# oxfordcontrol/Clarabel.rs

Measured on NVIDIA H100. Metric: ipm_iterations_per_sec, higher is better.
Workload: dtype f64

## Files before the change

clarabel.rs_b200/csrc/ldl.cu:

```cuda
#include <cuda_runtime.h>
#include <dlfcn.h>

#include <cmath>
#include <cstdio>
#include <cstring>
#include <algorithm>
#include <thread>
#include <vector>

#include "../../include/clarabel_b200.h"
#include "ldl_device.h"
#include "symbolic.h"
#include "vec.cuh"

namespace cb {

std::atomic<unsigned long long> g_launches{0};

typedef struct ncclComm* cb_ncclComm_t;
typedef struct { char internal[128]; } cb_ncclUniqueId;
struct NcclApi {
  void* lib = nullptr;
  int (*GetUniqueId)(cb_ncclUniqueId*) = nullptr;
  int (*CommInitRank)(cb_ncclComm_t*, int, cb_ncclUniqueId, int) = nullptr;
// ... 10 lines not shown
  void* h = dlopen(libpath && *libpath ? libpath : "libnccl.so.2", RTLD_NOW | RTLD_GLOBAL);
  if (!h) { std::fprintf(stderr, "[clarabel_b200] dlopen(%s) failed: %s\n", libpath ? libpath : "libnccl.so.2", dlerror()); return nullptr; }
  api.GetUniqueId = (int (*)(cb_ncclUniqueId*))dlsym(h, "ncclGetUniqueId");
  api.CommInitRank = (int (*)(cb_ncclComm_t*, int, cb_ncclUniqueId, int))dlsym(h, "ncclCommInitRank");
  api.AllGather = (int (*)(const void*, void*, size_t, int, cb_ncclComm_t, cudaStream_t))dlsym(h, "ncclAllGather");
  api.CommDestroy = (int (*)(cb_ncclComm_t))dlsym(h, "ncclCommDestroy");
  api.GetErrorString = (const char* (*)(int))dlsym(h, "ncclGetErrorString");
  if (!api.GetUniqueId || !api.CommInitRank || !api.AllGather || !api.CommDestroy) return nullptr;
  api.lib = h;
  return &api;
}



template <int NT>
__global__ void __launch_bounds__(NT) k_factor_level(LDLDev d, int task_base, int smem_cap) {
  extern __shared__ double sm[];
  __shared__ double s_inv;
  __shared__ double sD[CB_MAX_PANEL];
  const int tid = threadIdx.x;
  const int lane = tid & 31, warp = tid >> 5, nwarp = NT >> 5;
  const int s = d.level_tasks[task_base + blockIdx.x];
  const int f = d.sn_first[s];
  const int ns = d.sn_first[s + 1] - f;
  const long long rp = d.sn_rowptr[s];
  const int nr = (int)(d.sn_rowptr[s + 1] - rp);
  const int ld = ns + nr;
  double* __restrict__ P = d.L + d.panel_off[s];
  double* __restrict__ U = d.U + d.upd_off[s];
  const long long psz = (long long)ld * ns;
  const bool use_sm = psz <= (long long)smem_cap;
  double* W = use_sm ? sm : P;

  for (long long i = tid; i < psz; i += NT) W[i] = 0.0;
  for (int b = warp; b < nr; b += nwarp)
    for (int a = b + lane; a < nr; a += 32) U[(long long)b * nr + a] = 0.0;
  __syncthreads();

  for (long long e = d.asm_ptr[s] + tid; e < d.asm_ptr[s + 1]; e += NT)
    W[d.asm_dst[e]] = d.vals[d.asm_src[e]];
  __syncthreads();

  for (long long ci = d.child_ptr[s]; ci < d.child_ptr[s + 1]; ci++) {
    const int c = d.child_list[ci];
    const long long crp = d.sn_rowptr[c];
    const int nrc = (int)(d.sn_rowptr[c + 1] - crp);
    const double* __restrict__ Uc = d.U + d.upd_off[c];
    const int* __restrict__ relc = d.rel + crp;
    for (int b = warp; b < nrc; b += nwarp) {
      const int rb = relc[b];
      for (int a = b + lane; a < nrc; a += 32) {
        const int ra = relc[a];
        const double v = Uc[(long long)b * nrc + a];
        if (rb < ns) W[(long long)rb * ld + ra] += v;
        else U[(long long)(rb - ns) * nr + (ra - ns)] += v;
      }
    }
    __syncthreads();
  }

  for (int j = 0; j < ns; j++) {
    if (tid == 0) {
      double dj = W[(long long)j * ld + j];
      if (d.reg_enable) {
        const double sg = (double)d.dsigns[f + j];
        if (dj * sg < d.reg_eps) { dj = d.reg_delta * sg; atomicAdd(&d.status[ST_REGCOUNT], 1); }
      }
      if (dj == 0.0) atomicExch(&d.status[ST_ZEROPIV], 1);
      if (dj > 0.0) atomicAdd(&d.status[ST_POSINERTIA], 1);
      const double inv = 1.0 / dj;
      if (!isfinite(inv)) atomicExch(&d.status[ST_NONFINITE], 1);
      d.D[f + j] = dj;
      d.Dinv[f + j] = inv;
      W[(long long)j * ld + j] = dj;
      s_inv = inv;
      sD[j] = dj;
    }
    __syncthreads();
    const double inv = s_inv;
    const double* __restrict__ cj = W + (long long)j * ld;
    for (int k = j + 1 + warp; k < ns; k += nwarp) {
      const double wk = cj[k] * inv;
      double* __restrict__ ck = W + (long long)k * ld;
      for (int i = k + lane; i < ld; i += 32) ck[i] -= cj[i] * wk;
    }
    __syncthreads();
    double* cjw = W + (long long)j * ld;
    for (int i = j + 1 + tid; i < ld; i += NT) cjw[i] *= inv;
  }
  __syncthreads();

  for (int b = warp; b < nr; b += nwarp) {
    for (int a = b + lane; a < nr; a += 32) {
      double acc = 0.0;
      for (int k = 0; k < ns; k++) {
        const double* __restrict__ ck = W + (long long)k * ld + ns;
        acc += ck[a] * (ck[b] * sD[k]);
      }
      U[(long long)b * nr + a] -= acc;
    }
  }
  if (use_sm) {
    for (long long i = tid; i < psz; i += NT) P[i] = W[i];
  }
}

__global__ void __launch_bounds__(256) k_factor_leaf1(LDLDev d, int task_base, int count) {
  const int i = blockIdx.x * blockDim.x + threadIdx.x;
  const bool on = i < count;
  int pos = 0, reg = 0;
  if (on) {
    const int s = d.level_tasks[task_base + i];
    const int f = d.sn_first[s];
    const long long rp = d.sn_rowptr[s];
    const int nr = (int)(d.sn_rowptr[s + 1] - rp);
    const int ld = 1 + nr;
    double* __restrict__ P = d.L + d.panel_off[s];
    double* __restrict__ U = d.U + d.upd_off[s];
    for (int a = 0; a < ld; a++) P[a] = 0.0;
    for (long long e = d.asm_ptr[s]; e < d.asm_ptr[s + 1]; e++) P[d.asm_dst[e]] = d.vals[d.asm_src[e]];
    double dj = P[0];
    if (d.reg_enable) {
      const double sg = (double)d.dsigns[f];
      if (dj * sg < d.reg_eps) { dj = d.reg_delta * sg; reg = 1; }
    }
    if (dj == 0.0) atomicExch(&d.status[ST_ZEROPIV], 1);
    pos = dj > 0.0 ? 1 : 0;
    const double inv = 1.0 / dj;
    if (!isfinite(inv)) atomicExch(&d.status[ST_NONFINITE], 1);
    d.D[f] = dj;
    d.Dinv[f] = inv;
    P[0] = dj;
    for (int a = 1; a < ld; a++) P[a] *= inv;
    for (int b = 0; b < nr; b++) {
      const double t = P[1 + b] * dj;
      for (int a = b; a < nr; a++) {
        double acc = 0.0;
        acc += P[1 + a] * t;
        U[(long long)b * nr + a] = 0.0 - acc;
      }
    }
  }
  const unsigned mp = __ballot_sync(0xffffffffu, pos != 0), mr = __ballot_sync(0xffffffffu, reg != 0);
  if ((threadIdx.x & 31) == 0) {
    if (mp) atomicAdd(&d.status[ST_POSINERTIA], __popc(mp));
    if (mr) atomicAdd(&d.status[ST_REGCOUNT], __popc(mr));
  }
}

__global__ void k_permute_in(int n, const int* __restrict__ perm, const double* __restrict__ b,
                             double* __restrict__ xp) {
  int k = blockIdx.x * blockDim.x + threadIdx.x;
  if (k < n) xp[k] = b[perm[k]];
}

__device__ __forceinline__ unsigned long long df_gtime() {
#ifdef CB_EMU
  return 0;
#else
  unsigned long long t;
  asm volatile("mov.u64 %0, %%globaltimer;" : "=l"(t));
// ... 117 lines not shown
  if (tid == 0) {
    if (c_reg) atomicAdd(&d.status[ST_REGCOUNT], c_reg);
    if (c_pos) atomicAdd(&d.status[ST_POSINERTIA], c_pos);
    if (c_zero) atomicExch(&d.status[ST_ZEROPIV], 1);
    if (c_nonf) atomicExch(&d.status[ST_NONFINITE], 1);
  }
  for (int b = warp; b < nr; b += nwarp)
    for (int a = b + lane; a < nr; a += 32) {
      double acc = 0.0;
      for (int k = 0; k < ns; k++) {
        const double* ck = W + (long long)k * ld + ns;
        acc += ck[a] * (ck[b] * sD[k]);
      }
      U[(long long)b * nr + a] -= acc;
    }
  if (use_sm) for (long long i = tid; i < psz; i += DF_NT) P[i] = W[i];
}

#define DF_DCAP 32
#define DF_REC_INTS ((int)(sizeof(DFChildRec) / sizeof(int)))
#define DF_REC_INT(r, field) (reinterpret_cast<const int*>(r)[offsetof(DFChildRec, field) / sizeof(int)])

template <int NH>
__device__ __forceinline__ void df_add_child(const LDLDev& d, const DFChildRec& ch, double* dst, int rowoff,
                                             int rstride, int coloff, int cstride) {
  const int lane = threadIdx.x & 31, warp = threadIdx.x >> 5;
  const int* __restrict__ relc = d.rel + ch.relp;
  const double* Uc = d.U + ch.uoff;
  __syncwarp();
  if (ch.contig == 3) {
// ... 303 lines not shown
        if (jj < nj) {
          const double* lk = sA + (jb + jj) * CB_PB_LD + jb;
#pragma unroll
          for (int j2 = jj + 1; j2 < JB; j2++) t[j2] -= t[jj] * lk[j2];
        }
      }
#pragma unroll
      for (int jj = 0; jj < JB; jj++) if (jj < nj) prow[(jb + jj) * DF_RB] = t[jj] * sDinv[jb + jj];
    }
  }
  __syncthreads();
  const int nrow = r1 - r0;
  for (int idx = tid; idx < ns * DF_RB; idx += DF_NT) {
    const int j = idx / DF_RB, rr = idx - j * DF_RB;
    if (rr < nrow) P[(long long)j * ld + g0 + rr] = sR[idx];
  }
}

__device__ void dff_tile(const LDLDev& d, const DFFactor& q, const DFTask& tk, double* sm, int* s_desc, int* s_ed, double* s_ev) {
  double* sAt = sm;
  double* sBt = sm + TS * TS;
  double* sC = sm + 2 * TS * TS;
  double* sD = sC + TS * (TS + 1);
  const int tid = threadIdx.x;
  const int ti = tk.a, tj = tk.b, ns = tk.ns, nr = tk.nr, f = tk.f;
  const int ld = ns + nr;
  const double* P = d.L + tk.poff;
  double* U = d.U + tk.uoff;
  const int i0 = ti * TS, j0 = tj * TS;
  const int ni = min(TS, nr - i0), nj = min(TS, nr - j0);
// ... 134 lines not shown
#endif
      if (rr < ni && cc < nj && (i0 + rr >= j0 + cc))
        U[(long long)(j0 + cc) * nr + (i0 + rr)] = (use_sc ? creg[i][j] + sC[rr * (TS + 1) + cc] : creg[i][j]) - prod;
    }
  }
#undef OWN_R
#undef OWN_C
}

__global__ void __launch_bounds__(DF_NT, 2) k_factor_df(LDLDev d, DFFactor q) {
  extern __shared__ __align__(16) double dfsm[];
  __shared__ __align__(16) int s_desc[DF_DCAP * DF_REC_INTS];
  __shared__ __align__(16) int s_task[16];
  __shared__ int s_ed[DF_ENT_FAST];
  __shared__ double s_ev[DF_ENT_FAST];
  const int tid = threadIdx.x;
  if (tid == 0) df_cur_qi = -1;
  for (;;) {
    __syncthreads();
    if (tid == 0) {
      if (q.trace && df_cur_qi >= 0) q.trace[10 * (size_t)df_cur_qi + 2] = df_gtime();
      const int qi = atomicAdd(q.qhead, 1);
      df_cur_qi = qi < q.ntask ? qi : -1;
      if (q.trace && df_cur_qi >= 0) {
        unsigned smid = 0;
#ifndef CB_EMU
        asm volatile("mov.u32 %0, %%smid;" : "=r"(smid));
#endif
        q.trace[10 * (size_t)qi] = df_gtime();
        q.trace[10 * (size_t)qi + 3] = smid;
// ... 11 lines not shown
      __syncthreads();
      dff_small(d, s, dfsm, nullptr);
      __syncthreads();
      if (tid == 0) { __threadfence(); df_front_complete(q, s); }
    } else if (kind == 1) {
      if (tid == 0) { df_wait_zero(q.pend + s); __threadfence(); if (q.trace) q.trace[10 * (size_t)qi + 1] = df_gtime(); }
      __syncthreads();
      dff_diag(d, q, tk, dfsm, s_desc, s_ed, s_ev);
      __syncthreads();
      if (tid == 0) { __threadfence(); atomicExch(q.diag_done + s, 1); }
    } else if (kind == 2) {
      if (tid == 0) { df_wait_zero(q.pend + s); __threadfence(); if (q.trace) q.trace[10 * (size_t)qi + 1] = df_gtime(); }
      __syncthreads();
      dff_rows(d, q, tk, dfsm, s_desc, s_ed, s_ev);
      __syncthreads();
      if (tid == 0) { __threadfence(); atomicSub(q.rows_left + s, 1); }
    } else {
      if (tid == 0) { df_wait_zero(q.rows_left + s); __threadfence(); if (q.trace) q.trace[10 * (size_t)qi + 1] = df_gtime(); }
      __syncthreads();
      dff_tile(d, q, tk, dfsm, s_desc, s_ed, s_ev);
      __syncthreads();
      if (tid == 0) {
        __threadfence();
        if (atomicSub(q.tiles_left + s, 1) == 1) df_front_complete(q, s);
      }
    }
  }
}

__global__ void k_update_values(double* __restrict__ vals, const int* __restrict__ idx,
                                const double* __restrict__ v, long long len) {
// ... 159 lines not shown
  CK(upload(&dff.big_pos, fp.big_pos));
  CK(upload(&dff.tile_base, fp.tile_base));
  CK(cudaFuncSetAttribute(k_factor_df, cudaFuncAttributeMaxDynamicSharedMemorySize, DF_SMEM_DOUBLES * 8));
  int occ = 0;
  CK(cudaOccupancyMaxActiveBlocksPerMultiprocessor(&occ, k_factor_df, DF_NT, (size_t)DF_SMEM_DOUBLES * 8));
  dff_grid = nsm * std::max(1, occ);
  dff_nsup4 = 4 * (size_t)S.nsup;
  if (std::getenv("CB_DF_TRACE") && dff.ntask > 0) {
    h_dff_tasks = fp.tasks;
    CK(cudaMalloc((void**)&dff.trace, (size_t)dff.ntask * 10 * sizeof(unsigned long long)));
    CK(cudaMemset(dff.trace, 0, (size_t)dff.ntask * 10 * sizeof(unsigned long long)));
  }

  const int nt = (int)sp.tasks.size();
  sv_nwide = (int)sp.wide.size();
  sv_wide_runs = std::move(sp.wide_runs);
  sv_nleaf1 = (int)sp.leaf1.size(); sv_nleafn = (int)sp.leafn.size(); sv_nleafw = (int)sp.leafw.size();
  sv_leafw_nrmax = sp.leafw_nrmax;
  sv_leafw_grid = sv_nleafw;
  sv_ntask_owned = sp.ntask_owned;
  CK(upload(&dev.gat_ptr, sp.gat_ptr));
  CK(upload(&dev.gat_src, sp.gat_src));
  CK(upload(&d_sv_wide, sp.wide));
  CK(upload(&d_sv_leaf1, sp.leaf1));
  CK(upload(&d_sv_leafn, sp.leafn));
  CK(upload(&d_sv_leafw, sp.leafw));
  CK(upload(&sv.fronts, sp.fronts));
  CK(upload(&sv.front2task, sp.front2task));
  CK(upload(&sv.parent, S.sn_parent));
  CK(upload(&sv.tasks, sp.tasks));
  sv_ninit = sp.cnt_init.size();
  sv_nzero = (size_t)nt + 2 * (size_t)S.nsup + 2;
  CK(upload(&d_sv_init, sp.cnt_init));
  CK(cudaMalloc((void**)&d_sv_cnt, (sv_ninit + sv_nzero) * sizeof(int)));
  sv.pend = d_sv_cnt; sv.fleft = d_sv_cnt + nt; sv.bleft = sv.fleft + S.nsup;
  sv.tdone = d_sv_cnt + sv_ninit; sv.ydone = sv.tdone + nt; sv.done = sv.ydone + S.nsup; sv.qhead = sv.done + S.nsup;
  sv.bpart_stride = (long long)(sp.nslots ? sp.nslots : 1) * CB_PB_MAXNS;
  CK(cudaMalloc((void**)&sv.bpart, (size_t)2 * sv.bpart_stride * sizeof(double)));
// ... 28 lines not shown

void LDLObject::release() {
  cudaSetDevice(device);
  for (auto& w : d_shard_segs) for (auto& p : w) if (p) { cudaFree(p); p = nullptr; }
  for (int* p : d_shard_xidx) if (p) cudaFree(p);
  d_shard_xidx.clear();
  if (nccl_comm) { if (NcclApi* a = nccl_api(nullptr)) a->CommDestroy((cb_ncclComm_t)nccl_comm); nccl_comm = nullptr; }
  if (d_xsend) { cudaFree(d_xsend); d_xsend = nullptr; }
  if (d_xrecv) { cudaFree(d_xrecv); d_xrecv = nullptr; }
  xbuf_cap = 0;
  auto fr = [](const void* p) { if (p) cudaFree((void*)p); };
  fr(dev.sn_first); fr(dev.sn_rowptr); fr(dev.sn_rows); fr(dev.child_ptr); fr(dev.child_list);
  fr(dev.rel); fr(dev.panel_off); fr(dev.upd_off); fr(dev.asm_ptr); fr(dev.asm_src);
  fr(dev.asm_dst); fr(dev.level_tasks); fr(dev.perm); fr(dev.dsigns); fr(dev.vals); fr(dev.L);
  fr(dev.U); fr(dev.D); fr(dev.Dinv); fr(dev.u); fr(dev.status); fr(d_xp); fr(d_bx);
  fr(d_tmp_idx); fr(d_tmp_val); fr(d_tmp_sgn); fr(sv.tasks); fr(sv.fronts); fr(sv.front2task); fr(sv.parent); fr(sv.bpart); fr(sv.trace); fr(d_sv_cnt); fr(d_sv_init); fr(d_sv_wide); fr(d_sv_leaf1); fr(d_sv_leafn); fr(d_sv_leafw); fr(d_xp2); fr(d_u2); fr(dff.tasks); fr(dff.recs); fr(d_dff_init); fr(d_dff_cnt); fr(dff.qhead); fr(dff.parent); fr(dff.big_pos); fr(dff.tile_base); fr(dff.trace); fr(dev.gat_ptr); fr(dev.gat_src); fr(dev.sc_panel_src); fr(dev.sc_panel_dst); fr(dev.sc_tile_src); fr(dev.sc_tile_dst);
  if (h_status) cudaFreeHost(h_status);
  if (ev0) cudaEventDestroy(ev0);
  if (ev1) cudaEventDestroy(ev1);
  for (auto& e : ev_leaf) if (e) { cudaEventDestroy(e); e = nullptr; }
  if (stream_a) { cudaStreamDestroy(stream_a); stream_a = nullptr; }
  if (stream_b) { cudaStreamDestroy(stream_b); stream_b = nullptr; }
  if (stream) cudaStreamDestroy(stream);
}

int LDLObject::refactor_level0() {
  CK(cudaMemsetAsync(dev.status, 0, ST_COUNT * sizeof(int), stream));
  CK(cudaMemcpyAsync(d_dff_cnt, d_dff_init, dff_nsup4 * sizeof(int), cudaMemcpyDeviceToDevice, stream));
  CK(cudaMemsetAsync(dff.qhead, 0, sizeof(int), stream));
  g_launches += plan.size();
  for (const LaunchSeg& g : plan) {
    if (g.leaf1) k_factor_leaf1<<<(g.count + 255) / 256, 256, 0, stream>>>(dev, g.base, g.count);
    else if (g.threads == 64)
      k_factor_level<64><<<g.count, 64, (size_t)g.smem_doubles * 8, stream>>>(dev, g.base, g.smem_doubles);
    else
      k_factor_level<256><<<g.count, 256, (size_t)g.smem_doubles * 8, stream>>>(dev, g.base, g.smem_doubles);
  }
  return CLDL_OK;
}

int LDLObject::refactor_async() {
  if (sharded()) return has_transport() ? refactor_sharded() : CLDL_E_ARG;
  CK(cudaSetDevice(device));
  if (int rc = refactor_level0()) return rc;
  g_launches++;
  k_factor_df<<<dff_grid, DF_NT, (size_t)DF_SMEM_DOUBLES * 8, stream>>>(dev, dff);
  invert_pivots();
  CK(cudaGetLastError());
  CK(cudaMemcpyAsync(h_status, dev.status, ST_COUNT * sizeof(int), cudaMemcpyDeviceToHost, stream));
  factored = true;
  return CLDL_OK;
}

void LDLObject::invert_pivots() {
  if (!sv_nwide) return;
  g_launches++;
  for (size_t g = 0; g + 2 < sv_wide_runs.size(); g += 2) {
    const int first = sv_wide_runs[g], cnt = sv_wide_runs[g + 2] - first, ns = sv_wide_runs[g + 1];
    k_invert_pivots<<<cnt, 64, (size_t)ns * (ns + 1) * sizeof(double), stream>>>(dev, d_sv_wide + first, cnt);
  }
}

int LDLObject::sync_status() {
  CK(cudaSetDevice(device));
  CK(cudaStreamSynchronize(stream));
  regularize_count = (uint64_t)h_status[ST_REGCOUNT];
  positive_inertia = (uint64_t)h_status[ST_POSINERTIA];
  if (dff.trace) {
    std::vector<unsigned long long> tr((size_t)dff.ntask * 10);
    CK(cudaMemcpy(tr.data(), dff.trace, tr.size() * sizeof(unsigned long long), cudaMemcpyDeviceToHost));
    if (FILE* fp = std::fopen(std::getenv("CB_DF_TRACE"), "wb")) {
      const long long nt = dff.ntask;
      std::fwrite(&nt, sizeof(nt), 1, fp);
      std::fwrite(h_dff_tasks.data(), sizeof(DFTask), (size_t)nt, fp);
      std::fwrite(tr.data(), sizeof(unsigned long long), tr.size(), fp);
// ... 104 lines not shown
    q.ntask = dff_ntask_owned;
    g_launches++;
    k_factor_df<<<dff_grid, DF_NT, (size_t)DF_SMEM_DOUBLES * 8, stream>>>(dev, q);
    CK(cudaGetLastError());
    CK(cudaMemcpyAsync(h_status, dev.status, ST_COUNT * sizeof(int), cudaMemcpyDeviceToHost, stream));
    CK(cudaStreamSynchronize(stream));
    shard_count_owned[0] = (uint64_t)h_status[ST_REGCOUNT];
    shard_count_owned[1] = (uint64_t)h_status[ST_POSINERTIA];
    factored = false;
    return CLDL_OK;
  }
  h_phase_start[0] = dff_ntask_owned;
  CK(cudaMemcpyAsync(dff.qhead, &h_phase_start[0], sizeof(int), cudaMemcpyHostToDevice, stream));
  g_launches++;
  k_factor_df<<<dff_grid, DF_NT, (size_t)DF_SMEM_DOUBLES * 8, stream>>>(dev, dff);
  invert_pivots();
  CK(cudaGetLastError());
  CK(cudaMemcpyAsync(h_status, dev.status, ST_COUNT * sizeof(int), cudaMemcpyDeviceToHost, stream));
  factored = true;
  return CLDL_OK;
}

int LDLObject::solve_phase_async(double* d_x, const double* d_b, int phase) {
  if (!sharded()) return CLDL_E_ARG;
  if (!factored) return CLDL_E_NOT_FACTORED;
  CK(cudaSetDevice(device));
  SVPlan qv = sv;
  SVRhs r;
  r.xp[0] = r.xp[1] = d_xp; r.u[0] = r.u[1] = dev.u; r.out[0] = r.out[1] = d_x;
  if (phase == 0) {
    g_launches++;
// ... 300 lines not shown
  info->nnzL_stored = (uint64_t)o.S.nnzL_stored;
  info->regularize_count = o.regularize_count;
  info->positive_inertia = o.positive_inertia;
  info->n_supernodes = (uint64_t)o.S.nsup;
  info->n_levels = (uint64_t)o.S.nlevels;
  info->flops = o.S.flops_stored;
  info->ordering_used = o.S.ordering_used;
}

int cldl_get_perm(const cldl_t* h, uint64_t* perm_out) {
  if (!h || !perm_out) return CLDL_E_ARG;
  for (int k = 0; k < h->obj.n; k++) perm_out[k] = (uint64_t)h->obj.S.perm[k];
  return CLDL_OK;
}

int cldl_update_values_dev(cldl_t* h, const int32_t* d_index, const double* d_values, uint64_t len) {
  if (!h) return CLDL_E_ARG;
  if (len == 0) return CLDL_OK;
  LDLObject& o = h->obj;
  if (cudaSetDevice(o.device) != cudaSuccess) return CLDL_E_CUDA;
  cb::k_update_values<<<(unsigned)((len + 255) / 256), 256, 0, o.stream>>>(o.dev.vals, d_index, d_values, (long long)len);
  return CLDL_OK;
}

int cldl_set_values_dev(cldl_t* h, const double* d_nzval) {
  if (!h) return CLDL_E_ARG;
  LDLObject& o = h->obj;
  if (cudaSetDevice(o.device) != cudaSuccess) return CLDL_E_CUDA;
  return cudaMemcpyAsync(o.dev.vals, d_nzval, (size_t)o.nnzA * sizeof(double), cudaMemcpyDeviceToDevice, o.stream) == cudaSuccess
             ? CLDL_OK : CLDL_E_CUDA;
// ... 72 lines not shown
```

clarabel.rs_b200/csrc/ldl_device.h:

```cpp
#pragma once
#include <cuda_runtime.h>

#include <cstdint>
#include <cstdio>
#include <thread>
#include <vector>

#include "../../include/clarabel_b200.h"
#include "symbolic.h"
#include "ldl_plan.h"
#include "ldl_solve_plan.h"

#define CB_MAX_PANEL 128
#define CB_PB_LD 66

namespace cb {

struct ncclComm;

enum { ST_REGCOUNT = 0, ST_ZEROPIV = 1, ST_POSINERTIA = 2, ST_NONFINITE = 3, ST_COUNT = 8 };

struct LDLDev {
  const int* sn_first = nullptr;
  const long long* sn_rowptr = nullptr;
// ... 31 lines not shown
  int* pend = nullptr;
  int* diag_done = nullptr;
  int* rows_left = nullptr;
  int* tiles_left = nullptr;
  int* qhead = nullptr;
  const int* parent = nullptr;
  const int* big_pos = nullptr;
  const int* tile_base = nullptr;
  unsigned long long* trace = nullptr;
};


class LDLObject {
 public:
  SVPlan sv;
  int *d_sv_init = nullptr, *d_sv_cnt = nullptr, *d_sv_wide = nullptr, *d_sv_leaf1 = nullptr, *d_sv_leafn = nullptr, *d_sv_leafw = nullptr;
  size_t sv_ninit = 0, sv_nzero = 0, sv_smem[2] = {0, 0};
  int sv_cap = 0, sv_nwide = 0, sv_nleaf1 = 0, sv_nleafn = 0, sv_nleafw = 0, sv_leafw_nrmax = 0, sv_leafw_grid = 1, sv_ntask_owned = 0;
  std::vector<SVTask> h_sv_tasks;
  std::vector<int> sv_wide_runs;
  int sv_configure();
  int sv_occupancy();
  int sv_reset();
  void sv_sweep(bool fwd, int nrhs, const SVPlan& q, const SVRhs& r);
  void sv_leaves(bool fwd, int nrhs, const SVRhs& r);
  void invert_pivots();
  DFFactor dff;
  int *d_dff_init = nullptr, *d_dff_cnt = nullptr;
  std::vector<DFTask> h_dff_tasks;
  int dff_grid = 0;
  size_t dff_nsup4 = 0;
  int sv_grid = 0;
  bool use_dataflow = true;
  int n = 0;
  int64_t nnzA = 0;
  int device = 0;
  cldl_opts opts{};
  Symbolic S;
  LDLDev dev;
  std::vector<LaunchSeg> plan;
  std::thread big_alloc;
// ... 70 lines not shown
```

clarabel.rs_b200/csrc/ldl_plan.cpp:

```cpp
#include "ldl_plan.h"

#include <algorithm>
#include <thread>

namespace cb {

namespace {

int ns_of(const Symbolic& S, int s) { return S.sn_first[s + 1] - S.sn_first[s]; }
int nr_of(const Symbolic& S, int s) { return (int)(S.sn_rowptr[s + 1] - S.sn_rowptr[s]); }

bool is_big(const Symbolic& S, int s) { return nr_of(S, s) >= CB_BIG_NR && ns_of(S, s) <= CB_PB_MAXNS; }

std::vector<char> queued(const QueueOrder& q, int nsup) {
  std::vector<char> m(nsup, 0);
  for (const auto& ph : q)
    for (const auto& lev : ph)
      for (int s : lev) m[s] = 1;
  return m;
}

}

QueueOrder queue_order(const Symbolic& S, const std::vector<int>& owner, int rank) {
// ... 398 lines not shown
          t.dep0 = task_of_row(c, 0); t.dep1 = task_of_row(c, ns - 1);
          t.dep2 = t.r1 > 0 ? task_of_row(c, ns + t.r1 - 1) : t.dep1;
        } else {
          t.dep0 = task_of_row(c, ns + t.r0); t.dep1 = task_of_row(c, ns + t.r1 - 1);
        }
      }
    }
    P.nslots += nrt;
  }
  for (int s = 0; s < nsup; s++) {
    const int p = S.sn_parent[s];
    if (p >= 0 && f2t[s] >= 0 && chain_child[p] != s) pend[f2t[p]]++;
  }
  const std::vector<char> mine = queued(queue, nsup);
  for (int s = 0; s < nsup; s++) if (wide(s) && mine[s]) P.wide.push_back(s);
  std::stable_sort(P.wide.begin(), P.wide.end(), [&](int a, int b) { return ns_of(S, a) < ns_of(S, b); });
  const int nwide = (int)P.wide.size();
  const int bounds[] = {16, 24, 32, 40, 48, 56, CB_PB_MAXNS};
  int pos = 0;
  for (int bd : bounds) {
    int e = pos;
    while (e < nwide && ns_of(S, P.wide[e]) <= bd) e++;
    if (e > pos) { P.wide_runs.push_back(pos); P.wide_runs.push_back(bd); pos = e; }
  }
  P.wide_runs.push_back(nwide); P.wide_runs.push_back(0);
  return P;
}

}
```

clarabel.rs_b200/csrc/ldl_plan.h:

```cpp
#pragma once
#include <cstddef>
#include <cstdint>
#include <vector>

#include "symbolic.h"

#ifdef __CUDACC__
#define CB_HD __host__ __device__
#else
#define CB_HD
#endif

#define CB_PB_MAXNS 64
#define CB_SOLVE_SMALL_NS 8
#define CB_SMALL_CHILD 16
#define CB_BIG_NR 96
#define TS 64
#define DF_RB 128
#define SV_NT 256
#define SV_MAXROWS 256

namespace cb {

CB_HD inline int sv_lds(int srows, int ld) {
// ... 53 lines not shown
  std::vector<int> big_pos, tile_base;
  std::vector<int> sc_panel_ptr, sc_panel_src, sc_panel_dst, sc_tile_ptr, sc_tile_src, sc_tile_dst;
  std::vector<DFTask> tasks;
  std::vector<DFChildRec> recs;
  std::vector<int> cnt_init;
  int ntask_owned = 0;
};
FactorPlan build_factor_plan(const Symbolic& S, const std::vector<int>& owner, int rank);

struct SolvePlan {
  std::vector<SVTask> tasks;
  std::vector<int> cnt_init;
  std::vector<int> fronts, front2task;
  std::vector<int> leaf1, leafn, leafw;
  std::vector<int> wide;
  std::vector<int> wide_runs;
  std::vector<int> gat_ptr, gat_src;
  int nslots = 0, leafw_nrmax = 0;
  int ntask_owned = 0;
};
SolvePlan build_solve_plan(const Symbolic& S, const std::vector<int>& owner, int rank, int cap);

}
```

clarabel.rs_b200/csrc/ldl_solve.cuh:

```cuda
#pragma once

#include "ldl_solve_plan.h"

__device__ __forceinline__ void sv_cp8(double* smem_dst, const double* gsrc) {
#ifdef CB_EMU
  *smem_dst = *gsrc;
#else
  asm volatile("cp.async.ca.shared.global [%0], [%1], 8;" ::"r"((unsigned)__cvta_generic_to_shared(smem_dst)), "l"(gsrc) : "memory");
#endif
}
__device__ __forceinline__ void sv_cp16(double* smem_dst, const double* gsrc) {
#ifdef CB_EMU
  smem_dst[0] = gsrc[0]; smem_dst[1] = gsrc[1];
#else
  asm volatile("cp.async.cg.shared.global [%0], [%1], 16;" ::"r"((unsigned)__cvta_generic_to_shared(smem_dst)), "l"(gsrc) : "memory");
#endif
}
__device__ __forceinline__ void sv_mbar_init(unsigned long long* mbar) {
#ifndef CB_EMU
  asm volatile("mbarrier.init.shared::cta.b64 [%0], 1;" ::"r"((unsigned)__cvta_generic_to_shared(mbar)) : "memory");
  asm volatile("fence.proxy.async.shared::cta;" ::: "memory");
#endif
}
__device__ __forceinline__ void sv_bulk_load(double* smem_dst, const double* gsrc, unsigned bytes, unsigned long long* mbar) {
// ... 257 lines not shown
#pragma unroll
    for (int h = 0; h < NR; h++) {
      double t = acc[h];
#pragma unroll
      for (int o = 16; o > 0; o >>= 1) t += __shfl_xor_sync(0xffffffffu, t, o);
      if (lane == 0) s0[h * CB_PB_MAXNS + i] = st[h * CB_PB_MAXNS + i] + t;
    }
  }
  __syncthreads();
  if (tid < ns) {
    const int pf = d.perm[f + tid];
#pragma unroll
    for (int h = 0; h < NR; h++) { const double x = s0[h * CB_PB_MAXNS + tid]; r.xp[h][f + tid] = x; r.out[h][pf] = x; }
  }
  }
}

__global__ void __launch_bounds__(64) k_invert_pivots(LDLDev d, const int* __restrict__ wide, int count) {
  extern __shared__ double sA[];
  const int s = wide[blockIdx.x];
  const int f = d.sn_first[s];
  const int ns = d.sn_first[s + 1] - f;
  const int ld = ns + (int)(d.sn_rowptr[s + 1] - d.sn_rowptr[s]);
  double* __restrict__ P = d.L + d.panel_off[s];
  const int lane = threadIdx.x & 31, w = threadIdx.x >> 5;
  const int LDS = ns | 1;
  for (int j0 = 0; j0 < ns; j0 += 8) {
    double v[4][2];
#pragma unroll
    for (int c = 0; c < 4; c++) {
      const int j = j0 + 2 * c + w;
#pragma unroll
      for (int h = 0; h < 2; h++) {
        const int i = lane + 32 * h;
        v[c][h] = (j < ns && i > j && i < ns) ? P[(long long)j * ld + i] : 0.0;
      }
    }
#pragma unroll
    for (int c = 0; c < 4; c++) {
      const int j = j0 + 2 * c + w;
#pragma unroll
      for (int h = 0; h < 2; h++) {
        const int i = lane + 32 * h;
        if (j < ns && i > j && i < ns) sA[i * LDS + j] = v[c][h];
      }
    }
  }
  __syncthreads();
  if ((int)threadIdx.x < ns) {
    const int j = threadIdx.x;
    double* X = sA + j * LDS;
    for (int i = j + 1; i < ns; i++) {
      const double* Li = sA + i * LDS;
      double a0 = Li[j], a1 = 0.0;
      int k = j + 1;
      for (; k + 1 < i; k += 2) { a0 += Li[k] * X[k]; a1 += Li[k + 1] * X[k + 1]; }
      if (k < i) a0 += Li[k] * X[k];
      X[i] = -(a0 + a1);
    }
  }
  __syncthreads();
  for (int j = w; j < ns; j += 2)
    for (int i = j + 1 + lane; i < ns; i += 32) P[(long long)j * ld + i] = sA[j * LDS + i];
}

__device__ __forceinline__ int sv_ld_acquire(const int* p) {
#ifdef CB_EMU
  return *(volatile const int*)p;
#else
  int v;
  asm volatile("ld.acquire.gpu.global.s32 %0, [%1];" : "=r"(v) : "l"(p) : "memory");
  return v;
#endif
}
__device__ __forceinline__ void sv_set_release(int* p) {
#ifdef CB_EMU
  __threadfence(); atomicExch(p, 1);
#else
// ... 361 lines not shown
```

include/clarabel_b200.h:

```cpp
#ifndef CLARABEL_B200_H
#define CLARABEL_B200_H

#include <stdint.h>

#ifdef __cplusplus
extern "C" {
#endif

typedef struct cldl_handle cldl_t;

enum {
  CLDL_OK = 0,
  CLDL_E_DIM = -1,
  CLDL_E_EMPTY_COLUMN = -2,
  CLDL_E_NOT_TRIU = -3,
  CLDL_E_ZERO_PIVOT = -4,
  CLDL_E_BAD_PERM = -5,
  CLDL_E_CUDA = -20,
  CLDL_E_ARG = -21,
  CLDL_E_NOT_FACTORED = -22
};

enum { CLDL_ORDER_AMD = 1, CLDL_ORDER_ND = 2, CLDL_ORDER_BEST = 3 };

// ... 31 lines not shown
                const uint64_t *perm_or_null);
void cldl_destroy(cldl_t *h);

int cldl_update_values(cldl_t *h, const uint64_t *index, const double *values, uint64_t len);
int cldl_scale_values(cldl_t *h, const uint64_t *index, uint64_t len, double scale);
int cldl_offset_values(cldl_t *h, const uint64_t *index, uint64_t len, double offset,
                       const int8_t *signs);

int cldl_refactor(cldl_t *h);

int cldl_solve(cldl_t *h, double *x, const double *b);

void cldl_info(const cldl_t *h, cldl_info_t *info);

int cldl_get_perm(const cldl_t *h, uint64_t *perm_out);

int cldl_update_values_dev(cldl_t *h, const int32_t *d_index, const double *d_values, uint64_t len);
int cldl_set_values_dev(cldl_t *h, const double *d_nzval);
int cldl_refactor_dev(cldl_t *h);
int cldl_solve_dev(cldl_t *h, double *d_x, const double *d_b);
int cldl_sync_status(cldl_t *h);
void *cldl_stream(cldl_t *h);
double *cldl_values_dev(cldl_t *h);

int cldl_shard_refactor_phase_dev(cldl_t *h, int phase);
int cldl_shard_solve_phase_dev(cldl_t *h, double *d_x, const double *d_b, int phase);
uint64_t cldl_shard_count(const cldl_t *h, int what, int rank);
int cldl_shard_pack_dev(cldl_t *h, int what, double *d_buf, const double *d_x);
int cldl_shard_unpack_dev(cldl_t *h, int what, int rank, const double *d_buf, double *d_x);
int cldl_shard_counts(const cldl_t *h, uint64_t *out4);
// ... 147 lines not shown
```

Measured before the change: 25.10.

## Fuse pivot-block inversion into factor kernels and restructure leaf and level factorization

Removes the separate k_invert_pivots launch and its plan bookkeeping. The triangular pivot-block inverse is now computed inside the level kernel, the DF kernel and the last row-task of each DF supernode. The level kernel defers column scaling to a single pass, accumulates status flags locally, drops child extend-add and U zeroing, and blocks the Schur update over four columns. The leaf1 kernel moves from one thread per supernode to one warp per supernode using a shared-memory column buffer. The change also adds a cldl_get_factor export, and it assumes level tasks have no children.

```diff
diff --git a/clarabel.rs_b200/csrc/ldl.cu b/clarabel.rs_b200/csrc/ldl.cu
--- a/clarabel.rs_b200/csrc/ldl.cu
+++ b/clarabel.rs_b200/csrc/ldl.cu
@@ -48,10 +48,36 @@
 
 
 template <int NT>
+__device__ __forceinline__ void pivot_inverse(double* A, int lda, int ns) {
+  for (int j = threadIdx.x; j < ns; j += NT) {
+    for (int i = j + 1; i < ns; i++) {
+      double a0 = A[(long long)j * lda + i], a1 = 0.0;
+      int k = j + 1;
+      for (; k + 1 < i; k += 2) {
+        a0 += A[(long long)k * lda + i] * A[(long long)k * lda + j];
+        a1 += A[(long long)(k + 1) * lda + i] * A[(long long)(k + 1) * lda + j];
+      }
+      if (k < i) a0 += A[(long long)k * lda + i] * A[(long long)k * lda + j];
+      A[(long long)i * lda + j] = -(a0 + a1);
+    }
+  }
+}
+template <int NT>
+__device__ __forceinline__ void pivot_inverse_place(double* A, int lda, int ns) {
+  for (int idx = threadIdx.x; idx < ns * ns; idx += NT) {
+    const int j = idx / ns, i = idx - j * ns;
+    if (i > j) {
+      A[(long long)j * lda + i] = A[(long long)i * lda + j];
+      A[(long long)i * lda + j] = 0.0;
+    }
+  }
+}
+
+template <int NT>
 __global__ void __launch_bounds__(NT) k_factor_level(LDLDev d, int task_base, int smem_cap) {
   extern __shared__ double sm[];
-  __shared__ double s_inv;
   __shared__ double sD[CB_MAX_PANEL];
+  __shared__ double sInv[CB_MAX_PANEL];
   const int tid = threadIdx.x;
   const int lane = tid & 31, warp = tid >> 5, nwarp = NT >> 5;
   const int s = d.level_tasks[task_base + blockIdx.x];
@@ -67,83 +93,95 @@
   double* W = use_sm ? sm : P;
 
   for (long long i = tid; i < psz; i += NT) W[i] = 0.0;
-  for (int b = warp; b < nr; b += nwarp)
-    for (int a = b + lane; a < nr; a += 32) U[(long long)b * nr + a] = 0.0;
-  __syncthreads();
-
+  __syncthreads();
   for (long long e = d.asm_ptr[s] + tid; e < d.asm_ptr[s + 1]; e += NT)
     W[d.asm_dst[e]] = d.vals[d.asm_src[e]];
-  __syncthreads();
-
-  for (long long ci = d.child_ptr[s]; ci < d.child_ptr[s + 1]; ci++) {
-    const int c = d.child_list[ci];
-    const long long crp = d.sn_rowptr[c];
-    const int nrc = (int)(d.sn_rowptr[c + 1] - crp);
-    const double* __restrict__ Uc = d.U + d.upd_off[c];
-    const int* __restrict__ relc = d.rel + crp;
-    for (int b = warp; b < nrc; b += nwarp) {
-      const int rb = relc[b];
-      for (int a = b + lane; a < nrc; a += 32) {
-        const int ra = relc[a];
-        const double v = Uc[(long long)b * nrc + a];
-        if (rb < ns) W[(long long)rb * ld + ra] += v;
-        else U[(long long)(rb - ns) * nr + (ra - ns)] += v;
-      }
-    }
+
+  int c_reg = 0, c_pos = 0, c_zero = 0, c_nonf = 0;
+  for (int j = 0; j < ns; j++) {
     __syncthreads();
-  }
-
-  for (int j = 0; j < ns; j++) {
+    const double* __restrict__ cj = W + (long long)j * ld;
+    double dj = cj[j];
+    bool reg = false;
+    if (d.reg_enable) {
+      const double sg = (double)d.dsigns[f + j];
+      if (dj * sg < d.reg_eps) { dj = d.reg_delta * sg; reg = true; }
+    }
+    const double inv = 1.0 / dj;
     if (tid == 0) {
-      double dj = W[(long long)j * ld + j];
-      if (d.reg_enable) {
-        const double sg = (double)d.dsigns[f + j];
-        if (dj * sg < d.reg_eps) { dj = d.reg_delta * sg; atomicAdd(&d.status[ST_REGCOUNT], 1); }
-      }
-      if (dj == 0.0) atomicExch(&d.status[ST_ZEROPIV], 1);
-      if (dj > 0.0) atomicAdd(&d.status[ST_POSINERTIA], 1);
-      const double inv = 1.0 / dj;
-      if (!isfinite(inv)) atomicExch(&d.status[ST_NONFINITE], 1);
+      c_reg += reg ? 1 : 0;
+      c_pos += dj > 0.0 ? 1 : 0;
+      if (dj == 0.0) c_zero = 1;
+      if (!isfinite(inv)) c_nonf = 1;
       d.D[f + j] = dj;
       d.Dinv[f + j] = inv;
-      W[(long long)j * ld + j] = dj;
-      s_inv = inv;
       sD[j] = dj;
-    }
-    __syncthreads();
-    const double inv = s_inv;
-    const double* __restrict__ cj = W + (long long)j * ld;
+      sInv[j] = inv;
+    }
     for (int k = j + 1 + warp; k < ns; k += nwarp) {
       const double wk = cj[k] * inv;
       double* __restrict__ ck = W + (long long)k * ld;
       for (int i = k + lane; i < ld; i += 32) ck[i] -= cj[i] * wk;
     }
+  }
+  __syncthreads();
+  for (int j = warp; j < ns; j += nwarp) {
+    double* __restrict__ cj = W + (long long)j * ld;
+    const double inv = sInv[j];
+    if (lane == 0) cj[j] = sD[j];
+    for (int i = j + 1 + lane; i < ld; i += 32) cj[i] *= inv;
+  }
+  if (tid == 0) {
+    if (c_reg) atomicAdd(&d.status[ST_REGCOUNT], c_reg);
+    if (c_pos) atomicAdd(&d.status[ST_POSINERTIA], c_pos);
+    if (c_zero) atomicExch(&d.status[ST_ZEROPIV], 1);
+    if (c_nonf) atomicExch(&d.status[ST_NONFINITE], 1);
+  }
+  __syncthreads();
+
+  {
+    int it = 0;
+    for (int b0 = 0; b0 < nr; b0 += 4)
+      for (int a0 = b0; a0 < nr; a0 += 32, it++) {
+        if (it % nwarp != warp) continue;
+        const int a = a0 + lane;
+        const bool on = a < nr;
+        const int nb = min(4, nr - b0);
+        double acc[4] = {0.0, 0.0, 0.0, 0.0};
+        const double* __restrict__ ck = W + ns;
+        for (int k = 0; k < ns; k++, ck += ld) {
+          const double la = on ? ck[a] : 0.0, dk = sD[k];
+#pragma unroll
+          for (int c = 0; c < 4; c++) acc[c] += la * (ck[b0 + min(c, nb - 1)] * dk);
+        }
+#pragma unroll
+        for (int c = 0; c < 4; c++)
+          if (on && b0 + c < nr && a >= b0 + c) U[(long long)(b0 + c) * nr + a] = 0.0 - acc[c];
+      }
+  }
+  if (ns > CB_SOLVE_SMALL_NS) {
+    pivot_inverse<NT>(W, ld, ns);
     __syncthreads();
-    double* cjw = W + (long long)j * ld;
-    for (int i = j + 1 + tid; i < ld; i += NT) cjw[i] *= inv;
-  }
-  __syncthreads();
-
-  for (int b = warp; b < nr; b += nwarp) {
-    for (int a = b + lane; a < nr; a += 32) {
-      double acc = 0.0;
-      for (int k = 0; k < ns; k++) {
-        const double* __restrict__ ck = W + (long long)k * ld + ns;
-        acc += ck[a] * (ck[b] * sD[k]);
-      }
-      U[(long long)b * nr + a] -= acc;
-    }
+    pivot_inverse_place<NT>(W, ld, ns);
   }
   if (use_sm) {
+    __syncthreads();
     for (long long i = tid; i < psz; i += NT) P[i] = W[i];
   }
 }
 
-__global__ void __launch_bounds__(256) k_factor_leaf1(LDLDev d, int task_base, int count) {
-  const int i = blockIdx.x * blockDim.x + threadIdx.x;
-  const bool on = i < count;
-  int pos = 0, reg = 0;
-  if (on) {
+#define LEAF1_NT 256
+#define LEAF1_MAXLD 128
+static_assert(LEAF1_MAXLD > CB_BIG_NR, "a level-0 column must fit the per-warp buffer");
+__global__ void __launch_bounds__(LEAF1_NT) k_factor_leaf1(LDLDev d, int task_base, int count) {
+  __shared__ double s_col[LEAF1_NT / 32][LEAF1_MAXLD];
+  __shared__ int s_pos, s_reg;
+  const int lane = threadIdx.x & 31, warp = threadIdx.x >> 5;
+  const int i = blockIdx.x * (LEAF1_NT / 32) + warp;
+  if (threadIdx.x == 0) { s_pos = 0; s_reg = 0; }
+  __syncthreads();
+  if (i < count) {
+    double* col = s_col[warp];
     const int s = d.level_tasks[task_base + i];
     const int f = d.sn_first[s];
     const long long rp = d.sn_rowptr[s];
@@ -151,34 +189,46 @@
     const int ld = 1 + nr;
     double* __restrict__ P = d.L + d.panel_off[s];
     double* __restrict__ U = d.U + d.upd_off[s];
-    for (int a = 0; a < ld; a++) P[a] = 0.0;
-    for (long long e = d.asm_ptr[s]; e < d.asm_ptr[s + 1]; e++) P[d.asm_dst[e]] = d.vals[d.asm_src[e]];
-    double dj = P[0];
+    for (int a = lane; a < ld; a += 32) col[a] = 0.0;
+    __syncwarp();
+    for (long long e = d.asm_ptr[s] + lane; e < d.asm_ptr[s + 1]; e += 32) col[d.asm_dst[e]] = d.vals[d.asm_src[e]];
+    __syncwarp();
+    double dj = col[0];
+    bool reg = false;
     if (d.reg_enable) {
       const double sg = (double)d.dsigns[f];
-      if (dj * sg < d.reg_eps) { dj = d.reg_delta * sg; reg = 1; }
-    }
-    if (dj == 0.0) atomicExch(&d.status[ST_ZEROPIV], 1);
-    pos = dj > 0.0 ? 1 : 0;
+      if (dj * sg < d.reg_eps) { dj = d.reg_delta * sg; reg = true; }
+    }
     const double inv = 1.0 / dj;
-    if (!isfinite(inv)) atomicExch(&d.status[ST_NONFINITE], 1);
-    d.D[f] = dj;
-    d.Dinv[f] = inv;
-    P[0] = dj;
-    for (int a = 1; a < ld; a++) P[a] *= inv;
-    for (int b = 0; b < nr; b++) {
-      const double t = P[1 + b] * dj;
-      for (int a = b; a < nr; a++) {
+    if (lane == 0) {
+      if (dj == 0.0) atomicExch(&d.status[ST_ZEROPIV], 1);
+      if (!isfinite(inv)) atomicExch(&d.status[ST_NONFINITE], 1);
+      if (dj > 0.0) atomicAdd(&s_pos, 1);
+      if (reg) atomicAdd(&s_reg, 1);
+      d.D[f] = dj;
+      d.Dinv[f] = inv;
+    }
+    __syncwarp();
+    for (int a = lane; a < ld; a += 32) {
+      const double v = a == 0 ? dj : col[a] * inv;
+      col[a] = v;
+      P[a] = v;
+    }
+    __syncwarp();
+    for (int idx = lane; idx < nr * nr; idx += 32) {
+      const int b = idx / nr, a = idx - b * nr;
+      if (a >= b) {
+        const double t = col[1 + b] * dj;
         double acc = 0.0;
-        acc += P[1 + a] * t;
-        U[(long long)b * nr + a] = 0.0 - acc;
+        acc += col[1 + a] * t;
+        U[idx] = 0.0 - acc;
       }
     }
   }
-  const unsigned mp = __ballot_sync(0xffffffffu, pos != 0), mr = __ballot_sync(0xffffffffu, reg != 0);
-  if ((threadIdx.x & 31) == 0) {
-    if (mp) atomicAdd(&d.status[ST_POSINERTIA], __popc(mp));
-    if (mr) atomicAdd(&d.status[ST_REGCOUNT], __popc(mr));
+  __syncthreads();
+  if (threadIdx.x == 0) {
+    if (s_pos) atomicAdd(&d.status[ST_POSINERTIA], s_pos);
+    if (s_reg) atomicAdd(&d.status[ST_REGCOUNT], s_reg);
   }
 }
 
@@ -326,6 +376,12 @@
       }
       U[(long long)b * nr + a] -= acc;
     }
+  if (ns > CB_SOLVE_SMALL_NS) {
+    pivot_inverse<DF_NT>(W, ld, ns);
+    __syncthreads();
+    pivot_inverse_place<DF_NT>(W, ld, ns);
+    __syncthreads();
+  }
   if (use_sm) for (long long i = tid; i < psz; i += DF_NT) P[i] = W[i];
 }
 
@@ -659,6 +715,18 @@
   for (int idx = tid; idx < ns * DF_RB; idx += DF_NT) {
     const int j = idx / DF_RB, rr = idx - j * DF_RB;
     if (rr < nrow) P[(long long)j * ld + g0 + rr] = sR[idx];
+  }
+}
+
+__device__ void dff_rows_invert(const LDLDev& d, const DFTask& tk, double* sm) {
+  double* sA = sm;
+  const int ns = tk.ns, ld = ns + tk.nr;
+  double* P = d.L + tk.poff;
+  pivot_inverse<DF_NT>(sA, CB_PB_LD, ns);
+  __syncthreads();
+  for (int idx = threadIdx.x; idx < ns * ns; idx += DF_NT) {
+    const int j = idx / ns, i = idx - j * ns;
+    if (i > j) P[(long long)j * ld + i] = sA[i * CB_PB_LD + j];
   }
 }
 
@@ -823,6 +891,7 @@
   __shared__ __align__(16) int s_task[16];
   __shared__ int s_ed[DF_ENT_FAST];
   __shared__ double s_ev[DF_ENT_FAST];
+  __shared__ int s_last;
   const int tid = threadIdx.x;
   if (tid == 0) df_cur_qi = -1;
   for (;;) {
@@ -864,7 +933,9 @@
       __syncthreads();
       dff_rows(d, q, tk, dfsm, s_desc, s_ed, s_ev);
       __syncthreads();
-      if (tid == 0) { __threadfence(); atomicSub(q.rows_left + s, 1); }
+      if (tid == 0) { __threadfence(); s_last = atomicSub(q.rows_left + s, 1) == 1; }
+      __syncthreads();
+      if (s_last && tk.ns > CB_SOLVE_SMALL_NS) dff_rows_invert(d, tk, dfsm);
     } else {
       if (tid == 0) { df_wait_zero(q.rows_left + s); __threadfence(); if (q.trace) q.trace[10 * (size_t)qi + 1] = df_gtime(); }
       __syncthreads();
@@ -1054,14 +1125,12 @@
 
   const int nt = (int)sp.tasks.size();
   sv_nwide = (int)sp.wide.size();
-  sv_wide_runs = std::move(sp.wide_runs);
   sv_nleaf1 = (int)sp.leaf1.size(); sv_nleafn = (int)sp.leafn.size(); sv_nleafw = (int)sp.leafw.size();
   sv_leafw_nrmax = sp.leafw_nrmax;
   sv_leafw_grid = sv_nleafw;
   sv_ntask_owned = sp.ntask_owned;
   CK(upload(&dev.gat_ptr, sp.gat_ptr));
   CK(upload(&dev.gat_src, sp.gat_src));
-  CK(upload(&d_sv_wide, sp.wide));
   CK(upload(&d_sv_leaf1, sp.leaf1));
   CK(upload(&d_sv_leafn, sp.leafn));
   CK(upload(&d_sv_leafw, sp.leafw));
@@ -1120,7 +1189,7 @@
   fr(dev.rel); fr(dev.panel_off); fr(dev.upd_off); fr(dev.asm_ptr); fr(dev.asm_src);
   fr(dev.asm_dst); fr(dev.level_tasks); fr(dev.perm); fr(dev.dsigns); fr(dev.vals); fr(dev.L);
   fr(dev.U); fr(dev.D); fr(dev.Dinv); fr(dev.u); fr(dev.status); fr(d_xp); fr(d_bx);
-  fr(d_tmp_idx); fr(d_tmp_val); fr(d_tmp_sgn); fr(sv.tasks); fr(sv.fronts); fr(sv.front2task); fr(sv.parent); fr(sv.bpart); fr(sv.trace); fr(d_sv_cnt); fr(d_sv_init); fr(d_sv_wide); fr(d_sv_leaf1); fr(d_sv_leafn); fr(d_sv_leafw); fr(d_xp2); fr(d_u2); fr(dff.tasks); fr(dff.recs); fr(d_dff_init); fr(d_dff_cnt); fr(dff.qhead); fr(dff.parent); fr(dff.big_pos); fr(dff.tile_base); fr(dff.trace); fr(dev.gat_ptr); fr(dev.gat_src); fr(dev.sc_panel_src); fr(dev.sc_panel_dst); fr(dev.sc_tile_src); fr(dev.sc_tile_dst);
+  fr(d_tmp_idx); fr(d_tmp_val); fr(d_tmp_sgn); fr(sv.tasks); fr(sv.fronts); fr(sv.front2task); fr(sv.parent); fr(sv.bpart); fr(sv.trace); fr(d_sv_cnt); fr(d_sv_init); fr(d_sv_leaf1); fr(d_sv_leafn); fr(d_sv_leafw); fr(d_xp2); fr(d_u2); fr(dff.tasks); fr(dff.recs); fr(d_dff_init); fr(d_dff_cnt); fr(dff.qhead); fr(dff.parent); fr(dff.big_pos); fr(dff.tile_base); fr(dff.trace); fr(dev.gat_ptr); fr(dev.gat_src); fr(dev.sc_panel_src); fr(dev.sc_panel_dst); fr(dev.sc_tile_src); fr(dev.sc_tile_dst);
   if (h_status) cudaFreeHost(h_status);
   if (ev0) cudaEventDestroy(ev0);
   if (ev1) cudaEventDestroy(ev1);
@@ -1136,7 +1205,7 @@
   CK(cudaMemsetAsync(dff.qhead, 0, sizeof(int), stream));
   g_launches += plan.size();
   for (const LaunchSeg& g : plan) {
-    if (g.leaf1) k_factor_leaf1<<<(g.count + 255) / 256, 256, 0, stream>>>(dev, g.base, g.count);
+    if (g.leaf1) k_factor_leaf1<<<(g.count + LEAF1_NT / 32 - 1) / (LEAF1_NT / 32), LEAF1_NT, 0, stream>>>(dev, g.base, g.count);
     else if (g.threads == 64)
       k_factor_level<64><<<g.count, 64, (size_t)g.smem_doubles * 8, stream>>>(dev, g.base, g.smem_doubles);
     else
@@ -1151,20 +1220,10 @@
   if (int rc = refactor_level0()) return rc;
   g_launches++;
   k_factor_df<<<dff_grid, DF_NT, (size_t)DF_SMEM_DOUBLES * 8, stream>>>(dev, dff);
-  invert_pivots();
   CK(cudaGetLastError());
   CK(cudaMemcpyAsync(h_status, dev.status, ST_COUNT * sizeof(int), cudaMemcpyDeviceToHost, stream));
   factored = true;
   return CLDL_OK;
-}
-
-void LDLObject::invert_pivots() {
-  if (!sv_nwide) return;
-  g_launches++;
-  for (size_t g = 0; g + 2 < sv_wide_runs.size(); g += 2) {
-    const int first = sv_wide_runs[g], cnt = sv_wide_runs[g + 2] - first, ns = sv_wide_runs[g + 1];
-    k_invert_pivots<<<cnt, 64, (size_t)ns * (ns + 1) * sizeof(double), stream>>>(dev, d_sv_wide + first, cnt);
-  }
 }
 
 int LDLObject::sync_status() {
@@ -1299,7 +1358,6 @@
   CK(cudaMemcpyAsync(dff.qhead, &h_phase_start[0], sizeof(int), cudaMemcpyHostToDevice, stream));
   g_launches++;
   k_factor_df<<<dff_grid, DF_NT, (size_t)DF_SMEM_DOUBLES * 8, stream>>>(dev, dff);
-  invert_pivots();
   CK(cudaGetLastError());
   CK(cudaMemcpyAsync(h_status, dev.status, ST_COUNT * sizeof(int), cudaMemcpyDeviceToHost, stream));
   factored = true;
@@ -1630,6 +1688,25 @@
   return CLDL_OK;
 }
 
+int cldl_get_factor(const cldl_t* h, double* L_out, double* D_out, double* Dinv_out) {
+  if (!h || !L_out || !D_out || !Dinv_out) return CLDL_E_ARG;
+  const LDLObject& o = h->obj;
+  if (!o.factored) return CLDL_E_NOT_FACTORED;
+  if (cudaSetDevice(o.device) != cudaSuccess || cudaStreamSynchronize(o.stream) != cudaSuccess) return CLDL_E_CUDA;
+  std::vector<double> all((size_t)o.S.L_alloc);
+  if (cudaMemcpy(all.data(), o.dev.L, all.size() * sizeof(double), cudaMemcpyDeviceToHost) != cudaSuccess ||
+      cudaMemcpy(D_out, o.dev.D, (size_t)o.n * sizeof(double), cudaMemcpyDeviceToHost) != cudaSuccess ||
+      cudaMemcpy(Dinv_out, o.dev.Dinv, (size_t)o.n * sizeof(double), cudaMemcpyDeviceToHost) != cudaSuccess)
+    return CLDL_E_CUDA;
+  size_t pos = 0;
+  for (int s = 0; s < o.S.nsup; s++) {
+    const size_t ns = (size_t)(o.S.sn_first[s + 1] - o.S.sn_first[s]), nr = (size_t)(o.S.sn_rowptr[s + 1] - o.S.sn_rowptr[s]);
+    std::memcpy(L_out + pos, all.data() + o.S.panel_off[s], (ns + nr) * ns * sizeof(double));
+    pos += (ns + nr) * ns;
+  }
+  return CLDL_OK;
+}
+
 int cldl_update_values_dev(cldl_t* h, const int32_t* d_index, const double* d_values, uint64_t len) {
   if (!h) return CLDL_E_ARG;
   if (len == 0) return CLDL_OK;
diff --git a/clarabel.rs_b200/csrc/ldl_device.h b/clarabel.rs_b200/csrc/ldl_device.h
--- a/clarabel.rs_b200/csrc/ldl_device.h
+++ b/clarabel.rs_b200/csrc/ldl_device.h
@@ -69,17 +69,15 @@
 class LDLObject {
  public:
   SVPlan sv;
-  int *d_sv_init = nullptr, *d_sv_cnt = nullptr, *d_sv_wide = nullptr, *d_sv_leaf1 = nullptr, *d_sv_leafn = nullptr, *d_sv_leafw = nullptr;
+  int *d_sv_init = nullptr, *d_sv_cnt = nullptr, *d_sv_leaf1 = nullptr, *d_sv_leafn = nullptr, *d_sv_leafw = nullptr;
   size_t sv_ninit = 0, sv_nzero = 0, sv_smem[2] = {0, 0};
   int sv_cap = 0, sv_nwide = 0, sv_nleaf1 = 0, sv_nleafn = 0, sv_nleafw = 0, sv_leafw_nrmax = 0, sv_leafw_grid = 1, sv_ntask_owned = 0;
   std::vector<SVTask> h_sv_tasks;
-  std::vector<int> sv_wide_runs;
   int sv_configure();
   int sv_occupancy();
   int sv_reset();
   void sv_sweep(bool fwd, int nrhs, const SVPlan& q, const SVRhs& r);
   void sv_leaves(bool fwd, int nrhs, const SVRhs& r);
-  void invert_pivots();
   DFFactor dff;
   int *d_dff_init = nullptr, *d_dff_cnt = nullptr;
   std::vector<DFTask> h_dff_tasks;
diff --git a/clarabel.rs_b200/csrc/ldl_plan.cpp b/clarabel.rs_b200/csrc/ldl_plan.cpp
--- a/clarabel.rs_b200/csrc/ldl_plan.cpp
+++ b/clarabel.rs_b200/csrc/ldl_plan.cpp
@@ -436,16 +436,6 @@
   }
   const std::vector<char> mine = queued(queue, nsup);
   for (int s = 0; s < nsup; s++) if (wide(s) && mine[s]) P.wide.push_back(s);
-  std::stable_sort(P.wide.begin(), P.wide.end(), [&](int a, int b) { return ns_of(S, a) < ns_of(S, b); });
-  const int nwide = (int)P.wide.size();
-  const int bounds[] = {16, 24, 32, 40, 48, 56, CB_PB_MAXNS};
-  int pos = 0;
-  for (int bd : bounds) {
-    int e = pos;
-    while (e < nwide && ns_of(S, P.wide[e]) <= bd) e++;
-    if (e > pos) { P.wide_runs.push_back(pos); P.wide_runs.push_back(bd); pos = e; }
-  }
-  P.wide_runs.push_back(nwide); P.wide_runs.push_back(0);
   return P;
 }
 
diff --git a/clarabel.rs_b200/csrc/ldl_plan.h b/clarabel.rs_b200/csrc/ldl_plan.h
--- a/clarabel.rs_b200/csrc/ldl_plan.h
+++ b/clarabel.rs_b200/csrc/ldl_plan.h
@@ -91,7 +91,6 @@
   std::vector<int> fronts, front2task;
   std::vector<int> leaf1, leafn, leafw;
   std::vector<int> wide;
-  std::vector<int> wide_runs;
   std::vector<int> gat_ptr, gat_src;
   int nslots = 0, leafw_nrmax = 0;
   int ntask_owned = 0;
diff --git a/clarabel.rs_b200/csrc/ldl_solve.cuh b/clarabel.rs_b200/csrc/ldl_solve.cuh
--- a/clarabel.rs_b200/csrc/ldl_solve.cuh
+++ b/clarabel.rs_b200/csrc/ldl_solve.cuh
@@ -295,54 +295,6 @@
     for (int h = 0; h < NR; h++) { const double x = s0[h * CB_PB_MAXNS + tid]; r.xp[h][f + tid] = x; r.out[h][pf] = x; }
   }
   }
-}
-
-__global__ void __launch_bounds__(64) k_invert_pivots(LDLDev d, const int* __restrict__ wide, int count) {
-  extern __shared__ double sA[];
-  const int s = wide[blockIdx.x];
-  const int f = d.sn_first[s];
-  const int ns = d.sn_first[s + 1] - f;
-  const int ld = ns + (int)(d.sn_rowptr[s + 1] - d.sn_rowptr[s]);
-  double* __restrict__ P = d.L + d.panel_off[s];
-  const int lane = threadIdx.x & 31, w = threadIdx.x >> 5;
-  const int LDS = ns | 1;
-  for (int j0 = 0; j0 < ns; j0 += 8) {
-    double v[4][2];
-#pragma unroll
-    for (int c = 0; c < 4; c++) {
-      const int j = j0 + 2 * c + w;
-#pragma unroll
-      for (int h = 0; h < 2; h++) {
-        const int i = lane + 32 * h;
-        v[c][h] = (j < ns && i > j && i < ns) ? P[(long long)j * ld + i] : 0.0;
-      }
-    }
-#pragma unroll
-    for (int c = 0; c < 4; c++) {
-      const int j = j0 + 2 * c + w;
-#pragma unroll
-      for (int h = 0; h < 2; h++) {
-        const int i = lane + 32 * h;
-        if (j < ns && i > j && i < ns) sA[i * LDS + j] = v[c][h];
-      }
-    }
-  }
-  __syncthreads();
-  if ((int)threadIdx.x < ns) {
-    const int j = threadIdx.x;
-    double* X = sA + j * LDS;
-    for (int i = j + 1; i < ns; i++) {
-      const double* Li = sA + i * LDS;
-      double a0 = Li[j], a1 = 0.0;
-      int k = j + 1;
-      for (; k + 1 < i; k += 2) { a0 += Li[k] * X[k]; a1 += Li[k + 1] * X[k + 1]; }
-      if (k < i) a0 += Li[k] * X[k];
-      X[i] = -(a0 + a1);
-    }
-  }
-  __syncthreads();
-  for (int j = w; j < ns; j += 2)
-    for (int i = j + 1 + lane; i < ns; i += 32) P[(long long)j * ld + i] = sA[j * LDS + i];
 }
 
 __device__ __forceinline__ int sv_ld_acquire(const int* p) {
diff --git a/include/clarabel_b200.h b/include/clarabel_b200.h
--- a/include/clarabel_b200.h
+++ b/include/clarabel_b200.h
@@ -69,6 +69,8 @@
 void cldl_info(const cldl_t *h, cldl_info_t *info);
 
 int cldl_get_perm(const cldl_t *h, uint64_t *perm_out);
+
+int cldl_get_factor(const cldl_t *h, double *L_out, double *D_out, double *Dinv_out);
 
 int cldl_update_values_dev(cldl_t *h, const int32_t *d_index, const double *d_values, uint64_t len);
 int cldl_set_values_dev(cldl_t *h, const double *d_nzval);
```

Result: faster. 25.94 (median of 6 runs) (+3.3%).
